# AaronZ345/StyleSinger

Measured on AMD Instinct MI355X. Metric: mel-frames/sec (end-to-end infer incl. vocoder), higher is better.
Workload: dtype f32; 1 GPU; c2: batch=8x8.0s utterances per GPU (T=1500 frames, Tp=28, Tr=1500), 100 mel + 2x100 f0 diffusion steps + HiFi-GAN-NSF, exact fp32 MFMA; global_batch=8, frames_per_utterance=1500, parallelism=dp1, diffusion_loops=hipGraph replay, hipgraph_captures=6, frame_bucket=64, mfma_precision=fp32, step_overlap=3 HIP streams: consecutive batches run concurrently

## Files before the change

include/stylesinger_hip.h:

```cpp
#ifndef STYLESINGER_HIP_H
#define STYLESINGER_HIP_H

#include <stdint.h>

#ifdef __cplusplus
extern "C" {
#endif

#define SS_ABI_VERSION 20
#define SS_MAX_TAPS 16
#define SS_MAX_LAYERS 32

const char* ss_last_error(void);
int ss_abi_version(void);
int ss_device_info(int dev, int* n_cu, char* arch, int arch_len);
int ss_struct_sizes(int64_t* out, int n);
int ss_set_tuning(const char* key, int value);
int ss_get_tuning(const char* key);
int ss_set_clock_probe(void* dev_u64x2);
int ss_set_q4_guard(void* dev_u32x2);
int ss_debug_null_launch(int grid, int block, void* stream);

enum {
  SS_EPI_STORE = 0,
// ... 43 lines not shown
  int32_t ldc2;
  int64_t c2_batch_stride;
  int32_t Nh;
  float ddpm_recip, ddpm_recipm1, ddpm_c1, ddpm_c2, ddpm_sigma;
  const float* noise;
  uint64_t seed;
  const uint64_t* seed_dev;
  uint32_t step;
  int32_t tile;
  int32_t group_size;
  int64_t w_group_stride, bias_group_stride, a_bias_group_stride;
  int32_t mfma_bf16;
  int32_t ddpm_x0_pred;
  int32_t e_tiled;
  int32_t reserved2_;
} ss_conv_gemm_args;

int ss_conv_gemm(const ss_conv_gemm_args* args, void* stream);

int ss_gemm16_res(const ss_conv_gemm_args* args, int mt, void* stream);
int ss_gemm16_pick(int B, int T, int N);
int ss_gemm16_store(const ss_conv_gemm_args* args, int mt, void* stream);
int ss_gemm16_store_splitk(const ss_conv_gemm_args* args, int mt, int ksplit, float* partials, void* stream);
int ss_gemm16_ksplit_pick(int B, int T, int N, int K);

int ss_gemm16_resw(const ss_conv_gemm_args* args, const float* W16, int mt, void* stream);
int ss_pack_gemm16_weights(const float* src, float* dst, int Np, int Kp, void* stream);
int ss_wino43_gate16w(const ss_conv_gemm_args* args, const float* W16, int dilation, int mt, void* stream);
int ss_pack_gate16_weights(const float* src, float* dst, int Np, int Kp, void* stream);
int ss_wino43_gate16x(const ss_conv_gemm_args* args, const void* Wx, int dilation, int mt, void* stream);
int ss_split3_weights(const float* src, void* dst, int Np, int Kp, void* stream);
int ss_gemm16x_store(const ss_conv_gemm_args* args, const void* Wx, int mt, void* stream);
int ss_split3_gemm16_weights(const float* src, void* dst, int Np, int Kp, void* stream);
int64_t ss_split3_gemm16_elems(int Np, int Kp);
int ss_wino43_conv(const ss_conv_gemm_args* args, int k, int dilation, void* stream);
int ss_wino43_conv_ok(int C, int k, int dilation);
int ss_wino_gate(const ss_conv_gemm_args* args, int dilation, void* stream);
int ss_wino_weight_transform(const float* src, float* dst, int Cout, int Cin, void* stream);
int ss_wino43_gate(const ss_conv_gemm_args* args, int dilation, void* stream);
int ss_wino43_gate16(const ss_conv_gemm_args* args, int dilation, int mt, void* stream);
int ss_gate16_tile_addend(const float* E, int lde, int64_t e_batch_stride, float* E16, int B, int T, int Np, int dilation, int mt, void* stream);
int64_t ss_gate16_tiled_floats(int B, int T, int Np, int dilation, int mt);
int ss_wino43_gate16_pick(int B, int T, int Np, int dilation);
int ss_wino43_weight_transform(const float* src, float* dst, int Cout, int Cin, void* stream);

enum {
  SS_HEPI_STORE = 0,
  SS_HEPI_GATE = 1,
  SS_HEPI_RESX = 2
};
typedef struct ss_gemm_bf16_args {
  const uint16_t* A;
  int64_t a_batch_stride;
  int32_t lda;
  int32_t K;
// ... 186 lines not shown
  const uint16_t* w_dil_q[SS_MAX_LAYERS];
  int64_t gs_w_dil_q;
  float q_scale_gate;
  float q_scale_z;
  const uint16_t* w_skipall_q;
  int64_t gs_w_skipall_q;
  const uint16_t* w_dil_f[SS_MAX_LAYERS];
  const uint16_t* w_out_f[SS_MAX_LAYERS];
  int32_t n_wsets;
  int32_t mfma_products;
  int64_t ws_w_dil_h, ws_w_out_h, ws_w_skipall_h, ws_w_dil_f, ws_w_out_f;
  const uint16_t* w_skipall_c;
  int64_t ws_w_skipall_c;
  int32_t n_esets;
  int32_t reserved3_;
} ss_wavenet;

int64_t ss_wavenet_workspace_bytes(const ss_wavenet* net, int B, int T);

int ss_meldiff_sample(const ss_wavenet* net, float* x, const float* cond, const int32_t* lens, int B, int T,
                      const float* noise, uint64_t seed, const uint64_t* seed_dev, int step_lo, int step_hi,
                      int precompute_cond, void* ws, int64_t ws_bytes, void* stream);
int ss_meldiff_sample_ddim(const ss_wavenet* net, float* x, const float* cond, const int32_t* lens, int B, int T,
                           const int32_t* ts, int n_ts, const double* alphas_cumprod, float eta, const float* noise, uint64_t seed,
                           const uint64_t* seed_dev, int precompute_cond, void* ws, int64_t ws_bytes, void* stream);

int ss_meldiff_sample_plms(const ss_wavenet* net, float* x, const float* cond, const int32_t* lens, int B, int T, int step_hi, int interval,
                           const float* alphas_cumprod, int precompute, float* hist, void* ws, int64_t ws_bytes, void* stream);
int ss_prodiff_sample(const ss_wavenet* net, float* x, const float* cond, const int32_t* lens, int B, int T, const float* noise,
                      uint64_t seed, const uint64_t* seed_dev, int n_steps, const float* c1, const float* c2, const float* sigma,
// ... 99 lines not shown
```

stylesinger_amd/csrc/diffusion.hip:

```cpp
#include "common.h"
#include <stdlib.h>
#include "../../include/stylesinger_hip.h"

namespace {

inline int64_t align_up(int64_t x, int64_t a) { return (x + a - 1) / a * a; }
inline int round_up32(int x) { return (x + 31) / 32 * 32; }
constexpr int MTR = 2;

enum StackKind {
  STACK_FP32,
  STACK_PAIR16,
  STACK_FUSED16,
};
enum GateEntry { GATE_CONV, GATE_WINO23, GATE_WINO43, GATE_WINO43_16, GATE_WINO43_16W, GATE_WINO43_16X };
enum ProjEntry { PROJ_CONV, PROJ_RES16, PROJ_RES16W };
enum SkipEntry { SKIP_CONV, SKIP_STORE16, SKIP_SPLITK, SKIP_X3 };
struct LayerForm {
  int d;
  GateEntry gate;
  int mt;
  int64_t e16_floats;
  ProjEntry proj;
  bool q4_gate;
// ... 281 lines not shown
    a.W = net->w_dil[l];
    a.N = C;
    a.Np = 2 * C;
    a.Kp = round_up32(C);
    a.epi = SS_EPI_GATE;
    a.E = w.E + (int64_t)l * 2 * C;
    a.lde = NE;
    a.e_batch_stride = (int64_t)T * NE;
    float* Gl = sf.defer ? w.GA + (int64_t)l * C : w.G;
    set_c(a, Gl, ldg, T);
    a.mfma_bf16 = sf.conv_bf16;
    set_groups(a, net, B, net->gs_w_dil, 0, net->gs_dstep);
    if (y.gate != GATE_CONV) {
      a.W = net->w_dil_wino[l];
      a.w_group_stride = net->gs_w_dil_wino;
    }
    switch (y.gate) {
      case GATE_CONV: SS_PROPAGATE(ss_conv_gemm(&a, stream)); break;
      case GATE_WINO23: SS_PROPAGATE(ss_wino_gate(&a, y.d, stream)); break;
      case GATE_WINO43: SS_PROPAGATE(ss_wino43_gate(&a, y.d, stream)); break;
      case GATE_WINO43_16: SS_PROPAGATE(ss_wino43_gate16(&a, y.d, y.mt, stream)); break;
      case GATE_WINO43_16W:
        if (y.e16_floats) {
          a.E = w.E16[l];
          a.e_tiled = 1;
        }
        SS_PROPAGATE(ss_wino43_gate16w(&a, net->w_dil_wino16[l], y.d, y.mt, stream));
        break;
      case GATE_WINO43_16X:
        a.w_group_stride = net->gs_w_dil_x3;
// ... 840 lines not shown
```

stylesinger_amd/csrc/pack.hip:

```cpp
#include "common.h"
#include "../../include/stylesinger_hip.h"

namespace {

__device__ __forceinline__ int packed_to_orig(int np, int n, int interleave_half) {
  if (interleave_half > 0) {
    const int nb = np >> 5, jj = np & 31;
    const int p = nb >> 1, which = nb & 1;
    const int c = p * 32 + jj;
    return (c < interleave_half) ? which * interleave_half + c : -1;
  }
  return np < n ? np : -1;
}

__global__ void weight_norm_scale_kernel(const float* __restrict__ v, const float* __restrict__ g, float* scale, int rows,
                                         int cols) {
  const int r = blockIdx.x;
  if (r >= rows) return;
  float s = 0.f;
  for (int i = threadIdx.x; i < cols; i += blockDim.x) {
    const float x = v[(int64_t)r * cols + i];
    s += x * x;
  }
  __shared__ float red[4];
// ... 98 lines not shown
  const int grid = (int)((total + 255) / 256 < 4096 ? (total + 255) / 256 : 4096);
  hipLaunchKernelGGL(pack_convtr_kernel, dim3(grid), dim3(256), 0, (hipStream_t)stream, src, scale0, dst, Cin, Cout, k, u,
                     group, Np, Kp);
  SS_CHECK_LAUNCH("ss_pack_convtr_weight");
  return SS_OK;
}

extern "C" int ss_pack_bias(const float* src, const float* src2, float* dst, int n, int Np, int interleave_half,
                            int repeat, void* stream) {
  SS_CHECK_ARG(src && dst && n > 0 && Np > 0, "ss_pack_bias: bad args");
  hipLaunchKernelGGL(pack_bias_kernel, dim3((Np + 255) / 256), dim3(256), 0, (hipStream_t)stream, src, src2, dst, n, Np,
                     interleave_half, repeat);
  SS_CHECK_LAUNCH("ss_pack_bias");
  return SS_OK;
}
```

stylesinger_amd/csrc/wino43_gate16.hip:

```cpp
#include "common.h"
#include "device_prims.h"
#include "../../include/stylesinger_hip.h"
#include <type_traits>

namespace {

using namespace ss_dev;

constexpr int BK = 32;
constexpr int LD = BK;
constexpr int BN = 64;
constexpr int NC = 6;

__device__ __forceinline__ int lds_slot16(int row, int slot) { return row * LD + ((slot ^ swz16(row)) << 2); }

template <int MT, bool KS, bool WL>
__device__ __forceinline__ bool wino43_gate16_body(const ss_conv_gemm_args& a, const float* __restrict__ W16, int q_tiles_per_item, int q_tiles, int n_tiles,
                                                   int log2d, unsigned long long* clock_probe, const int block_id, float* __restrict__ smem_) {
  constexpr int BQ = 16 * MT;
  constexpr int NFULL = BQ / 32;
  constexpr bool HALF = (BQ % 32) != 0;
  const bool probing = clock_probe != nullptr && block_id == 0;
  unsigned long long probe_c0 = 0, probe_r0 = 0;
  if (probing) {
    probe_c0 = __builtin_readcyclecounter();
    probe_r0 = __builtin_amdgcn_s_memrealtime();
  }
  float* smem = static_cast<float*>(__builtin_assume_aligned(smem_, 16));
  float* As = smem;
  constexpr int SZC = BQ * LD;

// ... 29 lines not shown
  const int sh_c2 = tid & 15, sh_row = tid >> 4;
  int roff4[NFULL > 0 ? NFULL : 1][6];
  float mc4[NC][NFULL > 0 ? NFULL : 1];
  int roffh[6];
  float mch[NC];
  auto row_setup = [&](int q, int col_floats, int (&ro)[6], auto&& set_mc) {
    const int t = wino43_frame(q, d);
    float v[6];
#pragma unroll
    for (int r = 0; r < 6; ++r) {
      const int tr = t + (r - 1) * d;
      const bool ok = (unsigned)tr < (unsigned)len;
      v[r] = ok ? 1.0f : 0.0f;
      ro[r] = ok ? (tr * a.lda + col_floats) * 4 : (int)0x80000000;
    }
    set_mc(0, 4.f * v[0] - 5.f * v[2] + v[4]);
    set_mc(5, 4.f * v[1] - 5.f * v[3] + v[5]);
    set_mc(1, v[4] - 4.f * v[2]);
    set_mc(2, v[3] - 4.f * v[1]);
    set_mc(3, v[4] - v[2]);
    set_mc(4, v[3] - v[1]);
  };
#pragma unroll
  for (int i = 0; i < NFULL; ++i) row_setup(q0 + st_row + i * 32, st_c4 * 4, roff4[i], [&](int j, float x) { mc4[j][i] = x; });
  if constexpr (HALF) row_setup(q0 + NFULL * 32 + sh_row, sh_c2 * 2, roffh, [&](int j, float x) { mch[j] = x; });

  const int c7 = lc & 7, chi = lc >> 3;
  const int pc = n0 + 8 * wave + c7 + 32 * chi;
  const int w_voff = WL ? (nt * ldw * BN + wave * (ldw * BN / 4)) * 4 + lane * 16 : (pc * ldw + kg * 8) * 4;

  u32x4 rr4[NFULL > 0 ? NFULL : 1][6];
  u32x2 rr2[6];
  float4 rpb4;
  float2 rpb2;
  auto load_rows = [&](int ci0b) {
    ci0b = __builtin_amdgcn_readfirstlane(ci0b);
    if constexpr (NFULL > 0) rpb4 = __builtin_bit_cast(float4, __builtin_amdgcn_raw_buffer_load_b128(rsrc_bias, st_c4 * 16, ci0b, 0));
    if constexpr (HALF) rpb2 = __builtin_bit_cast(float2, __builtin_amdgcn_raw_buffer_load_b64(rsrc_bias, sh_c2 * 8, ci0b, 0));
#pragma unroll
    for (int i = 0; i < NFULL; ++i)
#pragma unroll
      for (int r = 0; r < 6; ++r) rr4[i][r] = __builtin_amdgcn_raw_buffer_load_b128(rsrc_a, roff4[i][r], ci0b, 0);
    if constexpr (HALF) {
#pragma unroll
      for (int r = 0; r < 6; ++r) rr2[r] = __builtin_amdgcn_raw_buffer_load_b64(rsrc_a, roffh[r], ci0b, 0);
    }
  };
  float4 bst[3][2];
  auto load_b = [&](auto stag, int comp, int k) {
    constexpr int S = decltype(stag)::value;
    if constexpr (WL) {
      const int cb = __builtin_amdgcn_readfirstlane(((k * NC + comp) * 2) * 1024);
      bst[S][0] = __builtin_bit_cast(float4, __builtin_amdgcn_raw_buffer_load_b128(rsrc_w, w_voff, cb, 0));
// ... 1 lines not shown
    } else {
      const int cb = __builtin_amdgcn_readfirstlane((comp * a.Kp + k * BK) * 4);
      bst[S][0] = __builtin_bit_cast(float4, __builtin_amdgcn_raw_buffer_load_b128(rsrc_w, w_voff, cb, 0));
      bst[S][1] = __builtin_bit_cast(float4, __builtin_amdgcn_raw_buffer_load_b128(rsrc_w, w_voff + 16, cb, 0));
    }
  };
  int a_wr4[NFULL > 0 ? NFULL : 1];
#pragma unroll
  for (int i = 0; i < NFULL; ++i) a_wr4[i] = lds_slot16(st_row + i * 32, st_c4);
  int a_wrh = lds_slot16(NFULL * 32 + sh_row, sh_c2 >> 1) + (sh_c2 & 1) * 2;
  float4 tA4[NFULL > 0 ? NFULL : 1], tB4[NFULL > 0 ? NFULL : 1], tC4[NFULL > 0 ? NFULL : 1], tD4[NFULL > 0 ? NFULL : 1];
  float2 tAh, tBh, tCh, tDh;
  auto build = [&](auto ptag, const auto& pb, float m0, float mA, float mB, float mC, float mD, float m5, const auto& r0, const auto& r1,
                   const auto& r2, const auto& r3, const auto& r4, const auto& r5, auto& tA, auto& tB, auto& tC, auto& tD) {
    constexpr int P = decltype(ptag)::value;
    if constexpr (P == 0) {
      tA = vfma(mA, pb, vfma(-4.f, r2, r4));
      tB = vfma(mB, pb, vfma(-4.f, r1, r3));
      return vadd(tA, tB);
    } else if constexpr (P == 1) {
      tC = vfma(mC, pb, vsub(r4, r2));
      return vfma(m0, pb, vfma(-5.f, r2, vfma(4.f, r0, r4)));
    } else if constexpr (P == 2) {
      tD = vfma(mD, pb, vsub(r3, r1));
      return vfma(m5, pb, vfma(-5.f, r3, vfma(4.f, r1, r5)));
    } else if constexpr (P == 3) {
      return vsub(tA, tB);
    } else if constexpr (P == 4) {
      return vfma(2.f, tD, tC);
    } else {
      return vfma(-2.f, tD, tC);
    }
  };
  auto store_a = [&](float* Ad, auto ptag) {
#pragma unroll
    for (int i = 0; i < NFULL; ++i) {
      auto R = [&](int q) { return __builtin_bit_cast(float4, rr4[i][q]); };
      const float4 v = build(ptag, rpb4, mc4[0][i], mc4[1][i], mc4[2][i], mc4[3][i], mc4[4][i], mc4[5][i], R(0), R(1), R(2), R(3), R(4),
                             R(5), tA4[i], tB4[i], tC4[i], tD4[i]);
      *reinterpret_cast<float4*>(Ad + a_wr4[i]) = v;
    }
    if constexpr (HALF) {
      auto R = [&](int q) { return __builtin_bit_cast(float2, rr2[q]); };
      const float2 v = build(ptag, rpb2, mch[0], mch[1], mch[2], mch[3], mch[4], mch[5], R(0), R(1), R(2), R(3), R(4), R(5), tAh, tBh, tCh, tDh);
      *reinterpret_cast<float2*>(Ad + a_wrh) = v;
    }
  };

  f32x4 acc[NC][MT];
#pragma unroll
  for (int j = 0; j < NC; ++j)
#pragma unroll
    for (int m = 0; m < MT; ++m)
#pragma unroll
      for (int r = 0; r < 4; ++r) acc[j][m][r] = 0.f;

  using P0 = std::integral_constant<int, 0>;
  using P1 = std::integral_constant<int, 1>;
  using P2 = std::integral_constant<int, 2>;
// ... 106 lines not shown
    }
  }
  {
  const int lane_e = __builtin_amdgcn_mbcnt_hi(~0u, __builtin_amdgcn_mbcnt_lo(~0u, 0u));
  const int lc = lane_e & 15, kg = lane_e >> 4;
  const int c7 = lc & 7, chi = lc >> 3;
  const int pc = n0 + 8 * wave + c7 + 32 * chi;
  const float* Eb = a.E ? a.E + (int64_t)b * a.e_batch_stride : nullptr;
  const __amdgpu_buffer_rsrc_t rsrc_e = __builtin_amdgcn_make_buffer_rsrc(
      uniform_ptr(Eb ? Eb : Wg), 0, __builtin_amdgcn_readfirstlane(Eb ? (int)((int64_t)a.T * a.lde * 4) : 0), 0x00020000);
  const int oc = (n0 >> 1) + 8 * wave + c7;
  const bool col_ok = oc < a.N;
  const int oob = col_ok ? 0 : (int)0x80000000;
  const int lde4 = a.lde * 4, ldc4 = a.ldc * 4;
  float pe[MT][4][4];
  auto fetch_addend = [&]() {
    if (a.e_tiled) {
      const __amdgpu_buffer_rsrc_t rsrc_t = __builtin_amdgcn_make_buffer_rsrc(
          uniform_ptr(a.E), 0, __builtin_amdgcn_readfirstlane((int)((int64_t)q_tiles * n_tiles * (MT * 4096) * 4)), 0x00020000);
      const int tile_b = __builtin_amdgcn_readfirstlane(((qt * n_tiles + nt) * (MT * 4096) + wave * (MT * 1024)) * 4);
#pragma unroll
      for (int m = 0; m < MT; ++m)
#pragma unroll
        for (int r = 0; r < 4; ++r) {
          const float4 v = __builtin_bit_cast(float4, __builtin_amdgcn_raw_buffer_load_b128(rsrc_t, lane_e * 16, tile_b + (m * 4 + r) * 1024, 0));
          pe[m][r][0] = v.x;
          pe[m][r][1] = v.y;
          pe[m][r][2] = v.z;
          pe[m][r][3] = v.w;
        }
      return;
// ... 33 lines not shown
  auto act = [&](float x) { return fmaf(__builtin_amdgcn_rcpf(1.0f + __builtin_amdgcn_exp2f(x * am)), as, ah); };
  auto partner = [](float x) {
    return __builtin_bit_cast(float, __builtin_amdgcn_mov_dpp(__builtin_bit_cast(int, x), 0x128, 0xf, 0xf, true));
  };
  const int row_lim = a.mask_rows ? (len < a.T ? len : a.T) : a.T;
  const int my_first = chi ? 2 * d : 0;
  auto epilogue = [&](auto fast_tag) {
    constexpr bool FAST = decltype(fast_tag)::value;
    float bs = 0.f;
    if constexpr (!FAST) bs = (a.bias && col_ok) ? a.bias[(int64_t)grp_w * a.bias_group_stride + pc] : 0.f;
#pragma unroll
    for (int m = 0; m < MT; ++m) {
      const int qm = q0 + 16 * m + 4 * kg;
      const int tm = wino43_frame(qm, d);
      const int c_base = (tm + my_first) * ldc4 + (oc * 4 + oob);
#pragma unroll
      for (int r = 0; r < 4; ++r) {
        const int dr = wino43_frame(r, d);
        const float a0 = acc[0][m][r], a5 = acc[5][m][r];
        float s12 = acc[1][m][r] + acc[2][m][r], d12 = acc[1][m][r] - acc[2][m][r];
        const float s34 = acc[3][m][r] + acc[4][m][r], d34 = acc[3][m][r] - acc[4][m][r];
        if constexpr (!FAST) {
          s12 += bs;
          d12 += bs;
        }
        const float z0 = a0 + s12 + s34;
        const float z1 = fmaf(2.0f, d34, d12);
        const float z2 = fmaf(4.0f, s34, s12);
        const float z3 = fmaf(8.0f, d34, d12) + a5;
        const float u0 = act(z0 + pe[m][r][0]);
        const float u1 = act(z1 + pe[m][r][1]);
        const float u2 = act(z2 + pe[m][r][2]);
        const float u3 = act(z3 + pe[m][r][3]);
        float g0, g1, g2, g3;
        g0 = u0 * partner(u0); g1 = u1 * partner(u1); g2 = u2 * partner(u2); g3 = u3 * partner(u3);
        float ga = chi ? g2 : g0, gb = chi ? g3 : g1;
        if constexpr (!FAST) {
          const int ta = tm + dr + my_first;
          if (ta >= row_lim) ga = 0.f;
          if (ta + d >= row_lim) gb = 0.f;
        }
        __builtin_amdgcn_raw_buffer_store_b32(__builtin_bit_cast(unsigned, ga), rsrc_c, c_base, dr * ldc4, 0);
        __builtin_amdgcn_raw_buffer_store_b32(__builtin_bit_cast(unsigned, gb), rsrc_c, c_base, (dr + d) * ldc4, 0);
      }
    }
  };
  const int q_last = q0 + BQ - 1;
  const bool fast = a.bias == nullptr && (wino43_frame(q_last, d) + 3 * d) < row_lim;
  if (fast) epilogue(std::true_type{});
  else epilogue(std::false_type{});
  }
  if (probing && wave == 0 && __builtin_amdgcn_mbcnt_lo(~0u, 0u) == 0 && __builtin_amdgcn_mbcnt_hi(~0u, 0u) == 0) {
    atomicAdd(clock_probe, (unsigned long long)__builtin_readcyclecounter() - probe_c0);
    atomicAdd(clock_probe + 1, (unsigned long long)__builtin_amdgcn_s_memrealtime() - probe_r0);
  }
  return true;
}

template <int MT, bool KS, bool WL>
__global__ __launch_bounds__(256, (MT <= 2 ? 3 : 2)) void wino43_gate16_kernel(const ss_conv_gemm_args a, const float* __restrict__ W16, int q_tiles_per_item,
                                                               int q_tiles, int n_tiles, int log2d, unsigned long long* clock_probe) {
  extern __shared__ __attribute__((aligned(16))) float smem[];
  wino43_gate16_body<MT, KS, WL>(a, W16, q_tiles_per_item, q_tiles, n_tiles, log2d, clock_probe, (int)blockIdx.x, smem);
}

template <int MT, bool KS, bool WL>
int launch16(const ss_conv_gemm_args& a, const float* W16, int dilation, int log2d, hipStream_t stream) {
  constexpr int BQ = 16 * MT;
  const int quads_per_item = ss_cdiv(a.T, 4 * dilation) * dilation;
  const int q_tiles_per_item = ss_cdiv(quads_per_item, BQ);
  const int q_tiles = q_tiles_per_item * a.B;
  const int n_tiles = a.Np / BN;
  const int grid = ss_cdiv(q_tiles, 8) * 8 * n_tiles;
  const size_t lds = (size_t)(KS ? 12 : 2) * BQ * LD * sizeof(float);
  if constexpr (KS && MT == 3) {
    const hipError_t attr = hipFuncSetAttribute(reinterpret_cast<const void*>(&wino43_gate16_kernel<MT, KS, WL>),
                                                hipFuncAttributeMaxDynamicSharedMemorySize, (int)lds);
    if (attr != hipSuccess) return (int)attr;
  }
  hipLaunchKernelGGL((wino43_gate16_kernel<MT, KS, WL>), dim3(grid), dim3(256), lds, stream, a, W16, q_tiles_per_item, q_tiles, n_tiles, log2d,
                     g_ss_tuning.clock_probe);
  return 0;
}

}

extern "C" int ss_wino43_gate16_pick(int B, int T, int Np, int dilation) {
  const int quads_per_item = ss_cdiv(T, 4 * dilation) * dilation;
  const int n_tiles = Np / BN;
  const int n_cu = ss_n_cu();
  auto layers = [&](int bq) { return ss_cdiv((long)ss_cdiv(quads_per_item, bq) * B * n_tiles, n_cu); };
  if (layers(64) >= 6) return 0;
  int best = 0;
  long best_cost = 4L * layers(64);
  const bool tiny = (long)ss_cdiv(quads_per_item, 32) * B * n_tiles <= n_cu;
// ... 54 lines not shown
}

int gate16_impl(const ss_conv_gemm_args* args, const float* W16, int dilation, int mt, void* stream, const char* who) {
  SS_CHECK_ARG(args != nullptr, "%s: null args", who);
  const ss_conv_gemm_args& a = *args;
  SS_CHECK_ARG(a.A && a.W && a.C, "%s: null A/W/C", who);
  SS_CHECK_ARG(dilation >= 1 && (dilation & (dilation - 1)) == 0 && dilation <= 64, "%s: dilation %d must be a power of two <= 64", who, dilation);
  SS_CHECK_ARG((a.Cin % BK) == 0 && a.Kp == a.Cin && (a.lda & 3) == 0, "%s: Cin=%d must be a multiple of 32 and Kp == Cin", who, a.Cin);
  SS_CHECK_ARG((a.Np % 64) == 0 && 2 * a.N <= a.Np, "%s: Np=%d must be a multiple of 64 and >= 2*N", who, a.Np);
  SS_CHECK_ARG((int64_t)a.T * a.lda * 4 < (1ll << 31) && (!a.E || (int64_t)a.T * a.lde * 4 < (1ll << 31)) &&
                   (int64_t)a.Np * NC * a.Kp * 4 < (1ll << 31),
               "%s: item too large for 32-bit offsets", who);
  SS_CHECK_ARG((int64_t)a.T * a.ldc * 4 < (1ll << 31), "%s: output item too large for 32-bit offsets", who);
  SS_CHECK_ARG(mt >= 0 && mt <= 3, "%s: mt=%d must be 0 (auto), 1, 2 or 3", who, mt);
  SS_CHECK_ARG(!a.e_tiled || (mt != 0 && a.E), "%s: a tiled addend (e_tiled) is laid out for ONE tiling: give mt explicitly", who);
  int log2d = 0;
  while ((1 << log2d) < dilation) ++log2d;
  const bool ks = g_ss_tuning.gate16_ks != 0 && a.Kp >= 2 * BK;
  if (mt == 0) {
    mt = ss_wino43_gate16_pick(a.B, a.T, a.Np, dilation);
    if (mt == 0) return ss_wino43_gate(args, dilation, stream);
    if (mt == 1 && !ks) mt = 2;
  }
  hipStream_t st = (hipStream_t)stream;
  int rc = 0;
  if (mt == 1) {
    SS_CHECK_ARG(ks, "%s: mt = 1 needs the K-staged form (Kp >= 64, gate16_ks on)", who);
    rc = W16 ? launch16<1, true, true>(a, W16, dilation, log2d, st) : launch16<1, true, false>(a, nullptr, dilation, log2d, st);
  } else if (W16) {
    if (mt == 2) rc = ks ? launch16<2, true, true>(a, W16, dilation, log2d, st) : launch16<2, false, true>(a, W16, dilation, log2d, st);
    else rc = ks ? launch16<3, true, true>(a, W16, dilation, log2d, st) : launch16<3, false, true>(a, W16, dilation, log2d, st);
  } else {
    if (mt == 2) rc = ks ? launch16<2, true, false>(a, nullptr, dilation, log2d, st) : launch16<2, false, false>(a, nullptr, dilation, log2d, st);
    else rc = ks ? launch16<3, true, false>(a, nullptr, dilation, log2d, st) : launch16<3, false, false>(a, nullptr, dilation, log2d, st);
  }
  SS_CHECK_ARG(rc == 0, "%s: hipFuncSetAttribute failed (%d)", who, rc);
  SS_CHECK_LAUNCH(who);
  return SS_OK;
}

}

extern "C" int ss_wino43_gate16(const ss_conv_gemm_args* args, int dilation, int mt, void* stream) {
  return gate16_impl(args, nullptr, dilation, mt, stream, "ss_wino43_gate16");
}

extern "C" int ss_wino43_gate16w(const ss_conv_gemm_args* args, const float* W16, int dilation, int mt, void* stream) {
  SS_CHECK_ARG(W16 != nullptr, "ss_wino43_gate16w: null W16");
  return gate16_impl(args, W16, dilation, mt, stream, "ss_wino43_gate16w");
}
// ... 32 lines not shown
```

stylesinger_amd/lib.py:

```python
import ctypes as C
import os
import re

import torch

HERE = os.path.dirname(os.path.abspath(__file__))
LIB_PATH = os.environ.get("SS_LIB_PATH") or os.path.join(HERE, "libstylesinger_hip.so")
HEADER = os.path.join(os.path.dirname(HERE), "include", "stylesinger_hip.h")

SS_MAX_TAPS = 16
SS_MAX_LAYERS = 32
SS_HG_MAX_UPS = 6
SS_HG_MAX_KERNELS = 4

ABI_VERSION = 20
EPI_STORE, EPI_GATE, EPI_RESSKIP, EPI_DDPM = 0, 1, 2, 3
ACT_NONE, ACT_RELU, ACT_GELU, ACT_MISH, ACT_TANH, ACT_LRELU = 0, 1, 2, 3, 4, 5

_fp = C.POINTER(C.c_float)
_vp = C.c_void_p


class StyleSingerHipError(RuntimeError):
    pass
# ... 3 lines not shown
    _fields_ = [
        ("A", _vp), ("a_batch_stride", C.c_int64), ("lda", C.c_int32), ("Cin", C.c_int32), ("ntaps", C.c_int32),
        ("tap_off", C.c_int32 * SS_MAX_TAPS), ("lens", _vp), ("B", C.c_int32), ("T", C.c_int32), ("a_bias", _vp),
        ("a_scale", C.c_float), ("a_lrelu", C.c_float),
        ("W", _vp), ("N", C.c_int32), ("Np", C.c_int32), ("Kp", C.c_int32),
        ("epi", C.c_int32), ("bias", _vp), ("pre_scale", C.c_float), ("act", C.c_int32), ("act_slope", C.c_float),
        ("E", _vp), ("lde", C.c_int32), ("e_batch_stride", C.c_int64), ("gate_mode", C.c_int32),
        ("R", _vp), ("ldr", C.c_int32), ("r_batch_stride", C.c_int64), ("post_scale", C.c_float),
        ("accumulate", C.c_int32), ("mask_rows", C.c_int32),
        ("C", _vp), ("ldc", C.c_int32), ("c_batch_stride", C.c_int64),
        ("C2", _vp), ("ldc2", C.c_int32), ("c2_batch_stride", C.c_int64), ("Nh", C.c_int32),
        ("ddpm_recip", C.c_float), ("ddpm_recipm1", C.c_float), ("ddpm_c1", C.c_float), ("ddpm_c2", C.c_float),
        ("ddpm_sigma", C.c_float), ("noise", _vp), ("seed", C.c_uint64), ("seed_dev", _vp), ("step", C.c_uint32), ("tile", C.c_int32),
        ("group_size", C.c_int32), ("w_group_stride", C.c_int64), ("bias_group_stride", C.c_int64), ("a_bias_group_stride", C.c_int64),
        ("mfma_bf16", C.c_int32), ("ddpm_x0_pred", C.c_int32), ("e_tiled", C.c_int32), ("reserved2_", C.c_int32),
    ]


class WaveNet(C.Structure):
    _fields_ = [
        ("C", C.c_int32), ("L", C.c_int32), ("cond_dim", C.c_int32), ("dil_cycle", C.c_int32), ("in_dim", C.c_int32),
        ("out_dim", C.c_int32), ("steps", C.c_int32),
        ("w_in", _vp), ("b_in", _vp), ("uv_embed", _vp), ("dstep", _vp),
        ("w_dil", _vp * SS_MAX_LAYERS), ("w_out", _vp * SS_MAX_LAYERS), ("b_out", _vp * SS_MAX_LAYERS),
        ("w_cond", _vp), ("b_cond", _vp), ("w_skip", _vp), ("b_skip", _vp), ("w_final", _vp), ("b_final", _vp),
        ("sqrt_recip_ac", _vp), ("sqrt_recipm1_ac", _vp), ("post_c1", _vp), ("post_c2", _vp), ("post_logvar", _vp),
        ("log_alpha", _vp), ("log_1m_alpha", _vp), ("log_cumprod_alpha", _vp), ("log_1m_cumprod_alpha", _vp),
        ("n_groups", C.c_int32), ("w_dil_wino", _vp * SS_MAX_LAYERS), ("gs_w_dil_wino", C.c_int64),
    ] + [(n, C.c_int64) for n in ("gs_w_in", "gs_b_in", "gs_uv_embed", "gs_dstep", "gs_w_dil", "gs_w_out", "gs_b_out", "gs_w_cond",
                                  "gs_b_cond", "gs_w_skip", "gs_b_skip", "gs_w_final", "gs_b_final")] \
        + [("mfma_bf16", C.c_int32), ("wino_m", C.c_int32), ("w_skipall", _vp), ("b_skipall", _vp),
           ("gs_w_skipall", C.c_int64), ("gs_b_skipall", C.c_int64), ("skipall_folded", C.c_int32), ("mfma_x3", C.c_int32),
           ("w_dil_h", _vp * SS_MAX_LAYERS), ("w_out_h", _vp * SS_MAX_LAYERS), ("w_skipall_h", _vp), ("w_cond_h", _vp),
           ("gs_w_dil_h", C.c_int64), ("gs_w_out_h", C.c_int64), ("gs_w_skipall_h", C.c_int64), ("gs_w_cond_h", C.c_int64),
           ("w_dil_x3", _vp * SS_MAX_LAYERS), ("gs_w_dil_x3", C.c_int64), ("w_dil_wino16", _vp * SS_MAX_LAYERS),
           ("w_out16", _vp * SS_MAX_LAYERS), ("gs_w_out16", C.c_int64), ("w_skipall_x3", _vp), ("gs_w_skipall_x3", C.c_int64),
           ("mfma_split", C.c_int32), ("mfma_out_scale", C.c_float),
           ("w_dil_q", _vp * SS_MAX_LAYERS), ("gs_w_dil_q", C.c_int64), ("q_scale_gate", C.c_float), ("q_scale_z", C.c_float),
           ("w_skipall_q", _vp), ("gs_w_skipall_q", C.c_int64),
           ("w_dil_f", _vp * SS_MAX_LAYERS), ("w_out_f", _vp * SS_MAX_LAYERS),
           ("n_wsets", C.c_int32), ("mfma_products", C.c_int32)] + [(n, C.c_int64) for n in ("ws_w_dil_h", "ws_w_out_h", "ws_w_skipall_h", "ws_w_dil_f", "ws_w_out_f")] \
        + [("w_skipall_c", _vp), ("ws_w_skipall_c", C.c_int64), ("n_esets", C.c_int32), ("reserved3_", C.c_int32)]


class GemmBf16Args(C.Structure):
    _fields_ = [
        ("A", _vp), ("a_batch_stride", C.c_int64), ("lda", C.c_int32), ("K", C.c_int32), ("ntaps", C.c_int32), ("tap_off", C.c_int32 * 4),
        ("lens", _vp), ("B", C.c_int32), ("T", C.c_int32), ("W", _vp), ("w_group_stride", C.c_int64), ("N", C.c_int32), ("Np", C.c_int32),
        ("epi", C.c_int32), ("act", C.c_int32), ("bias", _vp), ("bias_group_stride", C.c_int64), ("E", _vp), ("lde", C.c_int32),
        ("gate_mode", C.c_int32), ("e_batch_stride", C.c_int64), ("X", _vp), ("x_batch_stride", C.c_int64), ("ldx", C.c_int32),
        ("post_scale", C.c_float), ("next_bias", _vp), ("next_bias_group_stride", C.c_int64), ("Y", _vp), ("y_batch_stride", C.c_int64),
        ("ldy", C.c_int32), ("ldc", C.c_int32), ("C", _vp), ("c_batch_stride", C.c_int64), ("mask_rows", C.c_int32), ("group_size", C.c_int32),
        ("split", C.c_int32), ("out_scale", C.c_float), ("q_scale", C.c_float), ("one_product", C.c_int32), ("cur_bias", _vp), ("cur_bias_group_stride", C.c_int64),
        ("a_compact", C.c_int32), ("reserved2_", C.c_int32),
    ]


# ... 120 lines not shown
    return float(x)


def round_up(x, m):
    return (x + m - 1) // m * m


def conv_gemm(A, W, out, **kw):
    a = _fill_args(A, W, out, **kw)
    check(load().ss_conv_gemm(C.byref(a), stream_ptr()), "ss_conv_gemm")


def _fill_args(A, W, out, *, B, T, Cin, N, Np, Kp, lda=None, a_bs=None, taps=(0,), lens=None, a_bias=None, a_scale=1.0,
               a_lrelu=1.0, epi=EPI_STORE, bias=None, pre_scale=1.0, act=ACT_NONE, act_slope=0.0, E=None, lde=0, e_bs=0,
               gate_mode=0, R=None, ldr=0, r_bs=None, post_scale=1.0, accumulate=False, mask_rows=True, ldc=None, c_bs=None,
               C2=None, ldc2=0, c2_bs=0, Nh=0, tile=0, group_size=0, w_gs=0, bias_gs=0, a_bias_gs=0, bf16=False, e_tiled=False):
    a = ConvGemmArgs()
    a.A = ptr(A); a.lda = lda if lda is not None else Cin
    a.a_batch_stride = a_bs if a_bs is not None else T * a.lda
    a.Cin = Cin; a.ntaps = len(taps)
    for i, o in enumerate(taps):
        a.tap_off[i] = int(o)
    a.lens = ptr(lens); a.B = B; a.T = T; a.a_bias = ptr(a_bias); a.a_scale = a_scale; a.a_lrelu = a_lrelu
    a.W = ptr(W); a.N = N; a.Np = Np; a.Kp = Kp
    a.epi = epi; a.bias = ptr(bias); a.pre_scale = pre_scale; a.act = act; a.act_slope = act_slope
    a.E = ptr(E); a.lde = lde; a.e_batch_stride = e_bs; a.gate_mode = gate_mode
    a.R = ptr(R); a.ldr = ldr; a.r_batch_stride = r_bs if r_bs is not None else T * ldr
    a.post_scale = post_scale; a.accumulate = int(accumulate); a.mask_rows = int(mask_rows)
    a.C = ptr(out); a.ldc = ldc if ldc is not None else N
    a.c_batch_stride = c_bs if c_bs is not None else T * a.ldc
    a.C2 = ptr(C2); a.ldc2 = ldc2; a.c2_batch_stride = c2_bs; a.Nh = Nh; a.tile = tile
    a.group_size = group_size; a.w_group_stride = w_gs; a.bias_group_stride = bias_gs; a.a_bias_group_stride = a_bias_gs
    a.mfma_bf16 = 1 if bf16 else 0
    a.e_tiled = 1 if e_tiled else 0
    return a


def gate16_tile_addend(E, *, B, T, Np, lde, e_bs, dilation, mt):
    n = load().ss_gate16_tiled_floats(B, T, Np, int(dilation), int(mt))
    out = torch.empty(n, device=E.device, dtype=torch.float32)
    check(load().ss_gate16_tile_addend(ptr(E), lde, e_bs, ptr(out), B, T, Np, int(dilation), int(mt), stream_ptr()), "ss_gate16_tile_addend")
    return out


def wino_gate(A, Wt, out, *, dilation, **kw):
    kw.setdefault("epi", EPI_GATE)
    a = _fill_args(A, Wt, out, **kw)
    check(load().ss_wino_gate(C.byref(a), int(dilation), stream_ptr()), "ss_wino_gate")


def wino43_gate(A, Wt, out, *, dilation, **kw):
    kw.setdefault("epi", EPI_GATE)
    a = _fill_args(A, Wt, out, **kw)
    check(load().ss_wino43_gate(C.byref(a), int(dilation), stream_ptr()), "ss_wino43_gate")


def pack_gemm16_weights(Wp, Kp):
# ... 416 lines not shown
```

stylesinger_amd/model.py:

```python
import collections
import math

import numpy as np
import torch

from . import lib as L
from . import spec as _spec
from .config import make_hparams

_lib = L.load


class _Packed:
    __slots__ = ("W", "bias", "Cout", "Cin", "k", "Np", "Kp", "half")

    def __init__(self, W, bias, Cout, Cin, k, half=0):
        self.W, self.bias, self.Cout, self.Cin, self.k, self.half = W, bias, Cout, Cin, k, half
        self.Np, self.Kp = W.shape[0], W.shape[1] // k


def _sin_table(n, dim):
    half = dim // 2
    e = math.log(10000) / (half - 1)
    e = torch.exp(torch.arange(half, dtype=torch.float) * -e)
# ... 279 lines not shown
            bc_rows.append(cnd.bias)
        if self.defer_skip:
            wsk = torch.cat([self.p(f"{prefix}.residual_layers.{l}.output_projection.weight")[C:, :, 0] for l in range(Lyr)], dim=1)
            bsk = torch.stack([self.p(f"{prefix}.residual_layers.{l}.output_projection.bias")[C:] for l in range(Lyr)]).sum(0)
            if self.fold_skip:
                ws_ = self.p(prefix + ".skip_projection.weight")[:, :, 0].double()
                bs_ = self.p(prefix + ".skip_projection.bias").double()
                r = 1.0 / math.sqrt(Lyr)
                bsk = (ws_ @ bsk.double() * r + bs_).float()
                wsk = (ws_ @ wsk.double() * r).float()
            t["w_skipall"] = L.pack_conv_weight(wsk[:, :, None].contiguous())
            if self.x3 and self.fold_skip:
                t["w_skipall_x3"] = L.split3_gemm16_weights(t["w_skipall"], t["w_skipall"].shape[1])
            t["b_skipall"] = L.pack_bias(bsk.contiguous())
        t["dstep"] = dstep
        if self.f16 and not f0 and float(dstep.abs().max()) >= 16384.0:
            raise ValueError("mfma_precision=fp16x2: a diffusion-step embedding exceeds 16384 in magnitude - fp16 activations would overflow; use bf16x2")
        t["w_cond"] = torch.cat(wc_rows, 0).contiguous()
        t["b_cond"] = torch.cat(bc_rows, 0).contiguous()
        if self.bf16_hbm:
            t["w_cond_h"] = L.to_bf16(t["w_cond"])
            t["w_skipall_h"] = (self._sd_sets(t["w_skipall"]) if (self.sd and not f0) else self._split_w(t["w_skipall"], f0)) if self.split else L.to_bf16(t["w_skipall"])
            if self.sd and not f0 and t["w_skipall"].shape[1] % 64 == 0:
                t["w_skipall_c"] = L.split_planes(t["w_skipall_h"])[0].to(torch.float16).contiguous()
            if self.q4 and not f0 and t["w_skipall"].shape[1] % 64 == 0:
                t["w_skipall_q"] = L.pack_skip_q4(t["w_skipall"], shift=self.FP16_WSHIFT)[0]
        skip = self._pack_conv(prefix + ".skip_projection.weight", prefix + ".skip_projection.bias")
        fin = self._pack_conv(prefix + ".output_projection.weight", prefix + ".output_projection.bias")
        t["w_skip"], t["b_skip"], t["w_final"], t["b_final"] = skip.W, skip.bias, fin.W, fin.bias
        torch.cuda.synchronize()
# ... 37 lines not shown
            if self.use_wino:
                if f"w_dil_wino16.{l}" in packs[0]:
                    net.w_dil_wino16[l], _ = place(f"w_dil_wino16.{l}")
                if self.x3 and f"w_dil_x3.{l}" in packs[0]:
                    ptr_, gs = place(f"w_dil_x3.{l}")
                    net.w_dil_x3[l] = ptr_
                    net.gs_w_dil_x3 = gs
                    net.mfma_x3 = 1
            if self.bf16_hbm:
                for key, arr in (("w_dil_h", net.w_dil_h), ("w_out_h", net.w_out_h)):
                    ptr_, gs = place(f"{key}.{l}")
                    arr[l] = ptr_
                    setattr(net, "gs_" + key, gs)
        if "w_skipall_x3" in packs[0]:
            net.w_skipall_x3, net.gs_w_skipall_x3 = place("w_skipall_x3")
        if self.bf16_hbm:
            for key in ("w_cond_h", "w_skipall_h"):
                ptr_, gs = place(key)
                setattr(net, key, ptr_)
                setattr(net, "gs_" + key, gs)
        net.mfma_bf16 = 1 if self.bf16 else 0
        net.mfma_split = (2 if (self.f16 and not f0) else 1) if self.split else 0
        net.mfma_out_scale = 2.0 ** -self.FP16_WSHIFT if (self.f16 and not f0) else 1.0
        if self.sd and not f0:
            assert len(packs) == 1
            net.n_wsets, net.mfma_products = self.sd_sets, 1
            net.n_esets = self.sd_e_sets
            net.ws_w_dil_h, net.ws_w_out_h = packs[0]["w_dil_h.0"][0].numel(), packs[0]["w_out_h.0"][0].numel()
            net.ws_w_skipall_h = packs[0]["w_skipall_h"][0].numel()
            if "w_skipall_c" in packs[0]:
# ... 661 lines not shown
```

Measured before the change: 43570 mel-frames/s.

## Precompute per-step diffusion-embedding gate bias through dilated conv at pack time

Moves the per-step diffusion embedding term out of the Winograd gate kernel's input transform. A host-side table is built at weight-pack time holding the conv of each step embedding with the dilated weights, in four boundary variants (full, left-cut, right-cut, both). The kernel then skips the bias loads and the bias FMAs in its input build and adds the precomputed value in the epilogue, picking a variant per row near sequence edges. This trades fewer per-tile input-transform operations for an extra small table load, more template instantiations and boundary branching, and it applies only to the fp32 wino16 path.

```diff
diff --git a/include/stylesinger_hip.h b/include/stylesinger_hip.h
--- a/include/stylesinger_hip.h
+++ b/include/stylesinger_hip.h
@@ -81,6 +81,8 @@
   int32_t ddpm_x0_pred;
   int32_t e_tiled;
   int32_t reserved2_;
+  const float* step_bias;
+  int64_t step_bias_group_stride;
 } ss_conv_gemm_args;
 
 int ss_conv_gemm(const ss_conv_gemm_args* args, void* stream);
@@ -106,6 +108,7 @@
 int ss_wino_weight_transform(const float* src, float* dst, int Cout, int Cin, void* stream);
 int ss_wino43_gate(const ss_conv_gemm_args* args, int dilation, void* stream);
 int ss_wino43_gate16(const ss_conv_gemm_args* args, int dilation, int mt, void* stream);
+int ss_gate_step_bias_table(const float* w, const float* s, int rows, int64_t lds, int C, float* out, int64_t ldo);
 int ss_gate16_tile_addend(const float* E, int lde, int64_t e_batch_stride, float* E16, int B, int T, int Np, int dilation, int mt, void* stream);
 int64_t ss_gate16_tiled_floats(int B, int T, int Np, int dilation, int mt);
 int ss_wino43_gate16_pick(int B, int T, int Np, int dilation);
@@ -322,6 +325,8 @@
   int64_t ws_w_skipall_c;
   int32_t n_esets;
   int32_t reserved3_;
+  const float* step_bias;
+  int64_t gs_step_bias;
 } ss_wavenet;
 
 int64_t ss_wavenet_workspace_bytes(const ss_wavenet* net, int B, int T);
diff --git a/stylesinger_amd/csrc/diffusion.hip b/stylesinger_amd/csrc/diffusion.hip
--- a/stylesinger_amd/csrc/diffusion.hip
+++ b/stylesinger_amd/csrc/diffusion.hip
@@ -319,6 +319,10 @@
     if (y.gate != GATE_CONV) {
       a.W = net->w_dil_wino[l];
       a.w_group_stride = net->gs_w_dil_wino;
+    }
+    if (net->step_bias && (y.gate == GATE_WINO43_16 || y.gate == GATE_WINO43_16W)) {
+      a.step_bias = net->step_bias + ((int64_t)step * L + l) * 8 * C;
+      if (net->n_groups > 1) a.step_bias_group_stride = net->gs_step_bias;
     }
     switch (y.gate) {
       case GATE_CONV: SS_PROPAGATE(ss_conv_gemm(&a, stream)); break;
diff --git a/stylesinger_amd/csrc/pack.hip b/stylesinger_amd/csrc/pack.hip
--- a/stylesinger_amd/csrc/pack.hip
+++ b/stylesinger_amd/csrc/pack.hip
@@ -1,4 +1,5 @@
 #include "common.h"
+#include "step_bias_table.h"
 #include "../../include/stylesinger_hip.h"
 
 namespace {
@@ -136,3 +137,10 @@
   SS_CHECK_LAUNCH("ss_pack_bias");
   return SS_OK;
 }
+
+extern "C" int ss_gate_step_bias_table(const float* w, const float* s, int rows, int64_t lds, int C, float* out, int64_t ldo) {
+  SS_CHECK_ARG(w && s && out && rows > 0 && C > 0 && (C % 32) == 0 && lds >= C && ldo >= 8 * (int64_t)C,
+               "ss_gate_step_bias_table: C %% 32, lds >= C, ldo >= 8 C, host pointers");
+  ss_host::gate_step_bias_table(w, s, rows, lds, C, out, ldo);
+  return SS_OK;
+}
diff --git a/stylesinger_amd/csrc/step_bias_table.h b/stylesinger_amd/csrc/step_bias_table.h
--- /dev/null
+++ b/stylesinger_amd/csrc/step_bias_table.h
@@ -0,0 +1,38 @@
+#pragma once
+#include <cstddef>
+#include <cstdint>
+#include <vector>
+
+namespace ss_host {
+
+inline void gate_step_bias_table(const float* w, const float* s, int rows, int64_t lds, int C, float* out, int64_t ldo) {
+  const int N = 2 * C;
+  std::vector<double> wt((size_t)3 * C * N);
+  for (int n = 0; n < N; ++n)
+    for (int ci = 0; ci < C; ++ci)
+      for (int tap = 0; tap < 3; ++tap) wt[((size_t)tap * C + ci) * N + n] = (double)w[((size_t)n * C + ci) * 3 + tap];
+  std::vector<double> p((size_t)3 * N);
+  for (int r = 0; r < rows; ++r) {
+    const float* sr = s + (int64_t)r * lds;
+    for (size_t i = 0; i < p.size(); ++i) p[i] = 0.0;
+    for (int tap = 0; tap < 3; ++tap) {
+      double* pt = p.data() + (size_t)tap * N;
+      for (int ci = 0; ci < C; ++ci) {
+        const double x = (double)sr[ci];
+        const double* wr = wt.data() + ((size_t)tap * C + ci) * N;
+        for (int n = 0; n < N; ++n) pt[n] += wr[n] * x;
+      }
+    }
+    float* o = out + (int64_t)r * ldo;
+    for (int pc = 0; pc < N; ++pc) {
+      const int n = ((pc >> 5) & 1) * C + (pc >> 6) * 32 + (pc & 31);
+      const double left = p[n], mid = p[(size_t)N + n], right = p[(size_t)2 * N + n];
+      o[pc] = (float)(left + mid + right);
+      o[N + pc] = (float)(mid + right);
+      o[2 * N + pc] = (float)(left + mid);
+      o[3 * N + pc] = (float)mid;
+    }
+  }
+}
+
+}
diff --git a/stylesinger_amd/csrc/wino43_gate16.hip b/stylesinger_amd/csrc/wino43_gate16.hip
--- a/stylesinger_amd/csrc/wino43_gate16.hip
+++ b/stylesinger_amd/csrc/wino43_gate16.hip
@@ -14,7 +14,7 @@
 
 __device__ __forceinline__ int lds_slot16(int row, int slot) { return row * LD + ((slot ^ swz16(row)) << 2); }
 
-template <int MT, bool KS, bool WL>
+template <int MT, bool KS, bool WL, bool SB>
 __device__ __forceinline__ bool wino43_gate16_body(const ss_conv_gemm_args& a, const float* __restrict__ W16, int q_tiles_per_item, int q_tiles, int n_tiles,
                                                    int log2d, unsigned long long* clock_probe, const int block_id, float* __restrict__ smem_) {
   constexpr int BQ = 16 * MT;
@@ -74,12 +74,14 @@
       v[r] = ok ? 1.0f : 0.0f;
       ro[r] = ok ? (tr * a.lda + col_floats) * 4 : (int)0x80000000;
     }
-    set_mc(0, 4.f * v[0] - 5.f * v[2] + v[4]);
-    set_mc(5, 4.f * v[1] - 5.f * v[3] + v[5]);
-    set_mc(1, v[4] - 4.f * v[2]);
-    set_mc(2, v[3] - 4.f * v[1]);
-    set_mc(3, v[4] - v[2]);
-    set_mc(4, v[3] - v[1]);
+    if constexpr (!SB) {
+      set_mc(0, 4.f * v[0] - 5.f * v[2] + v[4]);
+      set_mc(5, 4.f * v[1] - 5.f * v[3] + v[5]);
+      set_mc(1, v[4] - 4.f * v[2]);
+      set_mc(2, v[3] - 4.f * v[1]);
+      set_mc(3, v[4] - v[2]);
+      set_mc(4, v[3] - v[1]);
+    }
   };
 #pragma unroll
   for (int i = 0; i < NFULL; ++i) row_setup(q0 + st_row + i * 32, st_c4 * 4, roff4[i], [&](int j, float x) { mc4[j][i] = x; });
@@ -95,8 +97,8 @@
   float2 rpb2;
   auto load_rows = [&](int ci0b) {
     ci0b = __builtin_amdgcn_readfirstlane(ci0b);
-    if constexpr (NFULL > 0) rpb4 = __builtin_bit_cast(float4, __builtin_amdgcn_raw_buffer_load_b128(rsrc_bias, st_c4 * 16, ci0b, 0));
-    if constexpr (HALF) rpb2 = __builtin_bit_cast(float2, __builtin_amdgcn_raw_buffer_load_b64(rsrc_bias, sh_c2 * 8, ci0b, 0));
+    if constexpr (NFULL > 0 && !SB) rpb4 = __builtin_bit_cast(float4, __builtin_amdgcn_raw_buffer_load_b128(rsrc_bias, st_c4 * 16, ci0b, 0));
+    if constexpr (HALF && !SB) rpb2 = __builtin_bit_cast(float2, __builtin_amdgcn_raw_buffer_load_b64(rsrc_bias, sh_c2 * 8, ci0b, 0));
 #pragma unroll
     for (int i = 0; i < NFULL; ++i)
 #pragma unroll
@@ -128,7 +130,17 @@
   auto build = [&](auto ptag, const auto& pb, float m0, float mA, float mB, float mC, float mD, float m5, const auto& r0, const auto& r1,
                    const auto& r2, const auto& r3, const auto& r4, const auto& r5, auto& tA, auto& tB, auto& tC, auto& tD) {
     constexpr int P = decltype(ptag)::value;
-    if constexpr (P == 0) {
+    if constexpr (SB && P == 0) {
+      tA = vfma(-4.f, r2, r4);
+      tB = vfma(-4.f, r1, r3);
+      return vadd(tA, tB);
+    } else if constexpr (SB && P == 1) {
+      tC = vsub(r4, r2);
+      return vfma(-5.f, r2, vfma(4.f, r0, r4));
+    } else if constexpr (SB && P == 2) {
+      tD = vsub(r3, r1);
+      return vfma(-5.f, r3, vfma(4.f, r1, r5));
+    } else if constexpr (P == 0) {
       tA = vfma(mA, pb, vfma(-4.f, r2, r4));
       tB = vfma(mB, pb, vfma(-4.f, r1, r3));
       return vadd(tA, tB);
@@ -150,13 +162,17 @@
 #pragma unroll
     for (int i = 0; i < NFULL; ++i) {
       auto R = [&](int q) { return __builtin_bit_cast(float4, rr4[i][q]); };
-      const float4 v = build(ptag, rpb4, mc4[0][i], mc4[1][i], mc4[2][i], mc4[3][i], mc4[4][i], mc4[5][i], R(0), R(1), R(2), R(3), R(4),
-                             R(5), tA4[i], tB4[i], tC4[i], tD4[i]);
+      float4 v;
+      if constexpr (SB) v = build(ptag, 0.f, 0.f, 0.f, 0.f, 0.f, 0.f, 0.f, R(0), R(1), R(2), R(3), R(4), R(5), tA4[i], tB4[i], tC4[i], tD4[i]);
+      else v = build(ptag, rpb4, mc4[0][i], mc4[1][i], mc4[2][i], mc4[3][i], mc4[4][i], mc4[5][i], R(0), R(1), R(2), R(3), R(4), R(5), tA4[i],
+                     tB4[i], tC4[i], tD4[i]);
       *reinterpret_cast<float4*>(Ad + a_wr4[i]) = v;
     }
     if constexpr (HALF) {
       auto R = [&](int q) { return __builtin_bit_cast(float2, rr2[q]); };
-      const float2 v = build(ptag, rpb2, mch[0], mch[1], mch[2], mch[3], mch[4], mch[5], R(0), R(1), R(2), R(3), R(4), R(5), tAh, tBh, tCh, tDh);
+      float2 v;
+      if constexpr (SB) v = build(ptag, 0.f, 0.f, 0.f, 0.f, 0.f, 0.f, 0.f, R(0), R(1), R(2), R(3), R(4), R(5), tAh, tBh, tCh, tDh);
+      else v = build(ptag, rpb2, mch[0], mch[1], mch[2], mch[3], mch[4], mch[5], R(0), R(1), R(2), R(3), R(4), R(5), tAh, tBh, tCh, tDh);
       *reinterpret_cast<float2*>(Ad + a_wrh) = v;
     }
   };
@@ -293,7 +309,15 @@
   const int oob = col_ok ? 0 : (int)0x80000000;
   const int lde4 = a.lde * 4, ldc4 = a.ldc * 4;
   float pe[MT][4][4];
+  float sbk[4] = {0.f, 0.f, 0.f, 0.f};
   auto fetch_addend = [&]() {
+    if constexpr (SB) {
+      const __amdgpu_buffer_rsrc_t rsrc_sb = __builtin_amdgcn_make_buffer_rsrc(
+          uniform_ptr(a.step_bias + (int64_t)grp_w * a.step_bias_group_stride), 0, __builtin_amdgcn_readfirstlane(4 * a.Np * 4), 0x00020000);
+#pragma unroll
+      for (int v = 0; v < 4; ++v)
+        sbk[v] = __builtin_bit_cast(float, __builtin_amdgcn_raw_buffer_load_b32(rsrc_sb, pc * 4 + oob, v * a.Np * 4, 0));
+    }
     if (a.e_tiled) {
       const __amdgpu_buffer_rsrc_t rsrc_t = __builtin_amdgcn_make_buffer_rsrc(
           uniform_ptr(a.E), 0, __builtin_amdgcn_readfirstlane((int)((int64_t)q_tiles * n_tiles * (MT * 4096) * 4)), 0x00020000);
@@ -357,6 +381,7 @@
       const int qm = q0 + 16 * m + 4 * kg;
       const int tm = wino43_frame(qm, d);
       const int c_base = (tm + my_first) * ldc4 + (oc * 4 + oob);
+      const int lm = (len - d) - tm;
 #pragma unroll
       for (int r = 0; r < 4; ++r) {
         const int dr = wino43_frame(r, d);
@@ -367,10 +392,22 @@
           s12 += bs;
           d12 += bs;
         }
-        const float z0 = a0 + s12 + s34;
-        const float z1 = fmaf(2.0f, d34, d12);
-        const float z2 = fmaf(4.0f, s34, s12);
-        const float z3 = fmaf(8.0f, d34, d12) + a5;
+        float z0 = a0 + s12 + s34;
+        float z1 = fmaf(2.0f, d34, d12);
+        float z2 = fmaf(4.0f, s34, s12);
+        float z3 = fmaf(8.0f, d34, d12) + a5;
+        if constexpr (SB && FAST) {
+          z0 += sbk[0];
+          z1 += sbk[0];
+          z2 += sbk[0];
+          z3 += sbk[0];
+        } else if constexpr (SB) {
+          const bool nl = tm + dr < d, nr0 = dr >= lm;
+          z0 += nl ? (nr0 ? sbk[3] : sbk[1]) : (nr0 ? sbk[2] : sbk[0]);
+          z1 += dr + d >= lm ? sbk[2] : sbk[0];
+          z2 += dr + 2 * d >= lm ? sbk[2] : sbk[0];
+          z3 += dr + 3 * d >= lm ? sbk[2] : sbk[0];
+        }
         const float u0 = act(z0 + pe[m][r][0]);
         const float u1 = act(z1 + pe[m][r][1]);
         const float u2 = act(z2 + pe[m][r][2]);
@@ -389,7 +426,7 @@
     }
   };
   const int q_last = q0 + BQ - 1;
-  const bool fast = a.bias == nullptr && (wino43_frame(q_last, d) + 3 * d) < row_lim;
+  const bool fast = a.bias == nullptr && (wino43_frame(q_last, d) + 3 * d) < row_lim && (!SB || (q0 >= d && wino43_frame(q_last, d) + 4 * d < len));
   if (fast) epilogue(std::true_type{});
   else epilogue(std::false_type{});
   }
@@ -400,14 +437,14 @@
   return true;
 }
 
-template <int MT, bool KS, bool WL>
+template <int MT, bool KS, bool WL, bool SB>
 __global__ __launch_bounds__(256, (MT <= 2 ? 3 : 2)) void wino43_gate16_kernel(const ss_conv_gemm_args a, const float* __restrict__ W16, int q_tiles_per_item,
                                                                int q_tiles, int n_tiles, int log2d, unsigned long long* clock_probe) {
   extern __shared__ __attribute__((aligned(16))) float smem[];
-  wino43_gate16_body<MT, KS, WL>(a, W16, q_tiles_per_item, q_tiles, n_tiles, log2d, clock_probe, (int)blockIdx.x, smem);
-}
-
-template <int MT, bool KS, bool WL>
+  wino43_gate16_body<MT, KS, WL, SB>(a, W16, q_tiles_per_item, q_tiles, n_tiles, log2d, clock_probe, (int)blockIdx.x, smem);
+}
+
+template <int MT, bool KS, bool WL, bool SB>
 int launch16(const ss_conv_gemm_args& a, const float* W16, int dilation, int log2d, hipStream_t stream) {
   constexpr int BQ = 16 * MT;
   const int quads_per_item = ss_cdiv(a.T, 4 * dilation) * dilation;
@@ -417,11 +454,11 @@
   const int grid = ss_cdiv(q_tiles, 8) * 8 * n_tiles;
   const size_t lds = (size_t)(KS ? 12 : 2) * BQ * LD * sizeof(float);
   if constexpr (KS && MT == 3) {
-    const hipError_t attr = hipFuncSetAttribute(reinterpret_cast<const void*>(&wino43_gate16_kernel<MT, KS, WL>),
+    const hipError_t attr = hipFuncSetAttribute(reinterpret_cast<const void*>(&wino43_gate16_kernel<MT, KS, WL, SB>),
                                                 hipFuncAttributeMaxDynamicSharedMemorySize, (int)lds);
     if (attr != hipSuccess) return (int)attr;
   }
-  hipLaunchKernelGGL((wino43_gate16_kernel<MT, KS, WL>), dim3(grid), dim3(256), lds, stream, a, W16, q_tiles_per_item, q_tiles, n_tiles, log2d,
+  hipLaunchKernelGGL((wino43_gate16_kernel<MT, KS, WL, SB>), dim3(grid), dim3(256), lds, stream, a, W16, q_tiles_per_item, q_tiles, n_tiles, log2d,
                      g_ss_tuning.clock_probe);
   return 0;
 }
@@ -506,6 +543,7 @@
   SS_CHECK_ARG((int64_t)a.T * a.ldc * 4 < (1ll << 31), "%s: output item too large for 32-bit offsets", who);
   SS_CHECK_ARG(mt >= 0 && mt <= 3, "%s: mt=%d must be 0 (auto), 1, 2 or 3", who, mt);
   SS_CHECK_ARG(!a.e_tiled || (mt != 0 && a.E), "%s: a tiled addend (e_tiled) is laid out for ONE tiling: give mt explicitly", who);
+  SS_CHECK_ARG(!a.step_bias || (a.mask_rows && a.a_bias), "%s: step_bias needs mask_rows and the a_bias it was built from", who);
   int log2d = 0;
   while ((1 << log2d) < dilation) ++log2d;
   const bool ks = g_ss_tuning.gate16_ks != 0 && a.Kp >= 2 * BK;
@@ -515,17 +553,18 @@
     if (mt == 1 && !ks) mt = 2;
   }
   hipStream_t st = (hipStream_t)stream;
+  SS_CHECK_ARG(mt != 1 || ks, "%s: mt = 1 needs the K-staged form (Kp >= 64, gate16_ks on)", who);
+  auto pick_sb = [&](auto mt_tag, auto ks_tag, auto wl_tag) {
+    constexpr int M = decltype(mt_tag)::value;
+    constexpr bool K = decltype(ks_tag)::value, WLF = decltype(wl_tag)::value;
+    return a.step_bias ? launch16<M, K, WLF, true>(a, W16, dilation, log2d, st) : launch16<M, K, WLF, false>(a, W16, dilation, log2d, st);
+  };
+  auto pick_wl = [&](auto mt_tag, auto ks_tag) { return W16 ? pick_sb(mt_tag, ks_tag, std::true_type{}) : pick_sb(mt_tag, ks_tag, std::false_type{}); };
+  auto pick_ks = [&](auto mt_tag) { return ks ? pick_wl(mt_tag, std::true_type{}) : pick_wl(mt_tag, std::false_type{}); };
   int rc = 0;
-  if (mt == 1) {
-    SS_CHECK_ARG(ks, "%s: mt = 1 needs the K-staged form (Kp >= 64, gate16_ks on)", who);
-    rc = W16 ? launch16<1, true, true>(a, W16, dilation, log2d, st) : launch16<1, true, false>(a, nullptr, dilation, log2d, st);
-  } else if (W16) {
-    if (mt == 2) rc = ks ? launch16<2, true, true>(a, W16, dilation, log2d, st) : launch16<2, false, true>(a, W16, dilation, log2d, st);
-    else rc = ks ? launch16<3, true, true>(a, W16, dilation, log2d, st) : launch16<3, false, true>(a, W16, dilation, log2d, st);
-  } else {
-    if (mt == 2) rc = ks ? launch16<2, true, false>(a, nullptr, dilation, log2d, st) : launch16<2, false, false>(a, nullptr, dilation, log2d, st);
-    else rc = ks ? launch16<3, true, false>(a, nullptr, dilation, log2d, st) : launch16<3, false, false>(a, nullptr, dilation, log2d, st);
-  }
+  if (mt == 1) rc = pick_wl(std::integral_constant<int, 1>{}, std::true_type{});
+  else if (mt == 2) rc = pick_ks(std::integral_constant<int, 2>{});
+  else rc = pick_ks(std::integral_constant<int, 3>{});
   SS_CHECK_ARG(rc == 0, "%s: hipFuncSetAttribute failed (%d)", who, rc);
   SS_CHECK_LAUNCH(who);
   return SS_OK;
diff --git a/stylesinger_amd/lib.py b/stylesinger_amd/lib.py
--- a/stylesinger_amd/lib.py
+++ b/stylesinger_amd/lib.py
@@ -41,6 +41,7 @@
         ("ddpm_sigma", C.c_float), ("noise", _vp), ("seed", C.c_uint64), ("seed_dev", _vp), ("step", C.c_uint32), ("tile", C.c_int32),
         ("group_size", C.c_int32), ("w_group_stride", C.c_int64), ("bias_group_stride", C.c_int64), ("a_bias_group_stride", C.c_int64),
         ("mfma_bf16", C.c_int32), ("ddpm_x0_pred", C.c_int32), ("e_tiled", C.c_int32), ("reserved2_", C.c_int32),
+        ("step_bias", _vp), ("step_bias_group_stride", C.c_int64),
     ]
 
 
@@ -67,7 +68,8 @@
            ("w_skipall_q", _vp), ("gs_w_skipall_q", C.c_int64),
            ("w_dil_f", _vp * SS_MAX_LAYERS), ("w_out_f", _vp * SS_MAX_LAYERS),
            ("n_wsets", C.c_int32), ("mfma_products", C.c_int32)] + [(n, C.c_int64) for n in ("ws_w_dil_h", "ws_w_out_h", "ws_w_skipall_h", "ws_w_dil_f", "ws_w_out_f")] \
-        + [("w_skipall_c", _vp), ("ws_w_skipall_c", C.c_int64), ("n_esets", C.c_int32), ("reserved3_", C.c_int32)]
+        + [("w_skipall_c", _vp), ("ws_w_skipall_c", C.c_int64), ("n_esets", C.c_int32), ("reserved3_", C.c_int32),
+           ("step_bias", _vp), ("gs_step_bias", C.c_int64)]
 
 
 class GemmBf16Args(C.Structure):
@@ -218,7 +220,8 @@
 def _fill_args(A, W, out, *, B, T, Cin, N, Np, Kp, lda=None, a_bs=None, taps=(0,), lens=None, a_bias=None, a_scale=1.0,
                a_lrelu=1.0, epi=EPI_STORE, bias=None, pre_scale=1.0, act=ACT_NONE, act_slope=0.0, E=None, lde=0, e_bs=0,
                gate_mode=0, R=None, ldr=0, r_bs=None, post_scale=1.0, accumulate=False, mask_rows=True, ldc=None, c_bs=None,
-               C2=None, ldc2=0, c2_bs=0, Nh=0, tile=0, group_size=0, w_gs=0, bias_gs=0, a_bias_gs=0, bf16=False, e_tiled=False):
+               C2=None, ldc2=0, c2_bs=0, Nh=0, tile=0, group_size=0, w_gs=0, bias_gs=0, a_bias_gs=0, bf16=False, e_tiled=False,
+               step_bias=None, step_bias_gs=0):
     a = ConvGemmArgs()
     a.A = ptr(A); a.lda = lda if lda is not None else Cin
     a.a_batch_stride = a_bs if a_bs is not None else T * a.lda
@@ -237,6 +240,7 @@
     a.group_size = group_size; a.w_group_stride = w_gs; a.bias_group_stride = bias_gs; a.a_bias_group_stride = a_bias_gs
     a.mfma_bf16 = 1 if bf16 else 0
     a.e_tiled = 1 if e_tiled else 0
+    a.step_bias = ptr(step_bias); a.step_bias_group_stride = step_bias_gs
     return a
 
 
@@ -245,6 +249,17 @@
     out = torch.empty(n, device=E.device, dtype=torch.float32)
     check(load().ss_gate16_tile_addend(ptr(E), lde, e_bs, ptr(out), B, T, Np, int(dilation), int(mt), stream_ptr()), "ss_gate16_tile_addend")
     return out
+
+
+def gate_step_bias_table(w, s):
+    import numpy as np
+    w = np.ascontiguousarray(w.detach().cpu().numpy() if torch.is_tensor(w) else w, dtype=np.float32)
+    s = np.ascontiguousarray(s.detach().cpu().numpy() if torch.is_tensor(s) else s, dtype=np.float32)
+    assert w.ndim == 3 and w.shape[2] == 3 and w.shape[0] == 2 * w.shape[1] and s.ndim == 2 and s.shape[1] == w.shape[1], (w.shape, s.shape)
+    Cc = w.shape[1]
+    out = np.empty((s.shape[0], 4, 2 * Cc), dtype=np.float32)
+    check(load().ss_gate_step_bias_table(hptr(w), hptr(s), s.shape[0], Cc, Cc, hptr(out), 4 * 2 * Cc), "ss_gate_step_bias_table")
+    return torch.from_numpy(out)
 
 
 def wino_gate(A, Wt, out, *, dilation, **kw):
diff --git a/stylesinger_amd/model.py b/stylesinger_amd/model.py
--- a/stylesinger_amd/model.py
+++ b/stylesinger_amd/model.py
@@ -317,6 +317,10 @@
                 t["w_skipall_x3"] = L.split3_gemm16_weights(t["w_skipall"], t["w_skipall"].shape[1])
             t["b_skipall"] = L.pack_bias(bsk.contiguous())
         t["dstep"] = dstep
+        if not self.bf16 and not self.x3 and all(f"w_dil_wino16.{l}" in t for l in range(Lyr)):
+            ds_host = dstep.cpu()
+            t["step_bias"] = torch.stack([L.gate_step_bias_table(self.p(f"{prefix}.residual_layers.{l}.dilated_conv.weight"), ds_host[:, l])
+                                          for l in range(Lyr)], dim=1).contiguous().to(dev)
         if self.f16 and not f0 and float(dstep.abs().max()) >= 16384.0:
             raise ValueError("mfma_precision=fp16x2: a diffusion-step embedding exceeds 16384 in magnitude - fp16 activations would overflow; use bf16x2")
         t["w_cond"] = torch.cat(wc_rows, 0).contiguous()
@@ -384,6 +388,8 @@
                     setattr(net, "gs_" + key, gs)
         if "w_skipall_x3" in packs[0]:
             net.w_skipall_x3, net.gs_w_skipall_x3 = place("w_skipall_x3")
+        if "step_bias" in packs[0]:
+            net.step_bias, net.gs_step_bias = place("step_bias")
         if self.bf16_hbm:
             for key in ("w_cond_h", "w_skipall_h"):
                 ptr_, gs = place(key)
```

New measurement: 43770 mel-frames/s (median of 6 runs). About the same (+0.5%).
